# summa-dev/halo2-experiments

Measured on AMD Instinct MI355X. Metric: BN256 G1 MSM throughput, higher is better.
Workload: dtype u32; 1 GPU; standalone BN256 G1 MSM, 2^24 points per GPU (global 2^24 x 1; BASELINE configs[4] microbench, north-star headline size); points_per_gpu=16777216, global_points=16777216, base_set=fixed-base table (registration default from 2^17 points), window_bits=22, windows=12, parallelism=index-range shards x1, all-gather of 96 B partials (RCCL) + host fold, base_set_bytes=12901679104

## Files before the change

halo2-experiments_amd/csrc/ff29.h:

```cpp
#pragma once
#include <stdint.h>

#if defined(__HIPCC__)
#define HM_HD __host__ __device__ __forceinline__
#else
#define HM_HD inline
#endif

#ifdef HM_BOUNDS
#include <cassert>
#include <cmath>
#include <cstdio>
#include <cstdlib>
#define HM_CHECK(cond, what)                                                        \
  do {                                                                              \
    if (!(cond)) {                                                                  \
      std::fprintf(stderr, "HM_BOUNDS violation: %s (%s:%d)\n", what, __FILE__, __LINE__); \
      std::abort();                                                                 \
    }                                                                               \
  } while (0)
#endif

namespace hm {

#include "bn256_constants.inc"

constexpr uint32_t MASK29 = (1u << 29) - 1u;

struct Arr9 {
  uint32_t v[9];
};

template <class F, int K, int BITS>
constexpr Arr9 make_sub_const() {
  Arr9 out{};
  uint64_t carry = 0;
  uint32_t c[9] = {};
  for (int i = 0; i < 9; ++i) {
    uint64_t t = (uint64_t)F::MOD[i] * (uint64_t)K + carry;
    if (i < 8) {
      c[i] = (uint32_t)(t & MASK29);
      carry = t >> 29;
    } else {
      c[i] = (uint32_t)t;
    }
  }
  const uint32_t b = 1u << (BITS - 29);
  out.v[0] = c[0] + (1u << BITS);
  for (int i = 1; i < 8; ++i) out.v[i] = c[i] + (1u << BITS) - b;
  out.v[8] = c[8] - b;
  return out;
}
template <class F, int K, int BITS>
struct SubConst {
  static constexpr Arr9 value = make_sub_const<F, K, BITS>();
};

template <class F>
struct Fe {
  uint32_t l[9];
#ifdef HM_BOUNDS
  double vb = 0;
  uint64_t lb = 0;
  uint64_t tb = 0;
#endif
};

#ifdef HM_BOUNDS
template <class F>
inline double mod_as_double() {
  double m = 0;
  for (int i = 8; i >= 0; --i) m = m * 536870912.0 + (double)F::MOD[i];
  return m;
}
template <class F>
inline uint64_t top_bound_from_value(double vb) {
  return (uint64_t)std::floor(vb * mod_as_double<F>() / std::ldexp(1.0, 232)) + 1;
}
template <class F>
inline void set_bounds(Fe<F>& a, double vb, uint64_t lb, uint64_t tb) {
  a.vb = vb; a.lb = lb; a.tb = tb;
  HM_CHECK(lb < (1ull << 32) && tb < (1ull << 32), "limb bound exceeds 32 bits");
  HM_CHECK(vb * mod_as_double<F>() < std::ldexp(1.0, 261), "value bound exceeds 2^261");
}
// ... 84 lines not shown
  }
#endif
  uint64_t t[10];
#pragma unroll
  for (int j = 0; j < 10; ++j) t[j] = 0;
#pragma unroll
  for (int i = 0; i < 9; ++i) {
#pragma unroll
    for (int j = 0; j < 9; ++j) t[j] += (uint64_t)a.l[j] * b.l[i];
#pragma unroll
    for (int j = 0; j < 9; ++j) t[j] += (uint64_t)c.l[j] * d.l[i];
    const uint32_t m = ((uint32_t)t[0] * F::INV29) & MASK29;
#pragma unroll
    for (int j = 0; j < 9; ++j) t[j] += (uint64_t)m * F::MOD[j];
    t[1] += t[0] >> 29;
#pragma unroll
    for (int j = 0; j < 9; ++j) t[j] = t[j + 1];
    t[9] = 0;
  }
  Fe<F> r;
#pragma unroll
  for (int j = 0; j < 8; ++j) {
    r.l[j] = (uint32_t)t[j] & MASK29;
    t[j + 1] += t[j] >> 29;
  }
  r.l[8] = (uint32_t)t[8];
#ifdef HM_BOUNDS
  {
    double vb = (a.vb * b.vb + c.vb * d.vb) * mod_as_double<F>() / std::ldexp(1.0, 261) + 1.0;
    set_bounds(r, vb, MASK29, top_bound_from_value<F>(vb));
    HM_CHECK(r.l[8] <= r.tb, "fe_mul2 result exceeds its bound");
  }
#endif
  return r;
}

template <class F>
HM_HD Fe<F> fe_sqr(const Fe<F>& a) {
#ifdef HM_BOUNDS
  {
    long double A = (long double)(a.lb > a.tb ? a.lb : a.tb);
    HM_CHECK(2.0L * A < 4294967296.0L, "fe_sqr doubled limb overflows");
    HM_CHECK(9.0L * A * A + 9.0L * 288230376151711744.0L + 1099511627776.0L < 18446744073709551616.0L,
             "fe_sqr column sum may overflow 64 bits");
  }
#endif
  uint32_t d[9];
#pragma unroll
  for (int j = 0; j < 9; ++j) d[j] = a.l[j] << 1;
  uint64_t t[10];
#pragma unroll
  for (int j = 0; j < 10; ++j) t[j] = 0;
#pragma unroll
  for (int i = 0; i < 9; ++i) {
    if (2 * i - i <= 8) t[i] += (uint64_t)a.l[i] * a.l[i];
#pragma unroll
    for (int j = i + 1; j < 9; ++j)
      if (j <= 8) t[j] += (uint64_t)a.l[i] * d[j];
    const uint32_t m = ((uint32_t)t[0] * F::INV29) & MASK29;
#pragma unroll
    for (int j = 0; j < 9; ++j) t[j] += (uint64_t)m * F::MOD[j];
    t[1] += t[0] >> 29;
#pragma unroll
    for (int j = 0; j < 9; ++j) t[j] = t[j + 1];
    t[9] = 0;
  }
  Fe<F> r;
#pragma unroll
  for (int j = 0; j < 8; ++j) {
    r.l[j] = (uint32_t)t[j] & MASK29;
    t[j + 1] += t[j] >> 29;
  }
  r.l[8] = (uint32_t)t[8];
#ifdef HM_BOUNDS
  {
    double vb = a.vb * a.vb * mod_as_double<F>() / std::ldexp(1.0, 261) + 1.0;
    set_bounds(r, vb, MASK29, top_bound_from_value<F>(vb));
    HM_CHECK(r.l[8] <= r.tb, "fe_sqr result exceeds its bound");
  }
#endif
  return r;
}

template <class F>
HM_HD Fe<F> fe_add(const Fe<F>& a, const Fe<F>& b) {
  Fe<F> r;
#pragma unroll
  for (int i = 0; i < 9; ++i) r.l[i] = a.l[i] + b.l[i];
#ifdef HM_BOUNDS
  set_bounds(r, a.vb + b.vb, a.lb + b.lb, a.tb + b.tb);
#endif
  return r;
}

template <class F>
HM_HD Fe<F> fe_dbl(const Fe<F>& a) { return fe_add(a, a); }

template <class F>
HM_HD Fe<F> fe_mul4(const Fe<F>& a) {
  Fe<F> r;
#pragma unroll
  for (int i = 0; i < 9; ++i) r.l[i] = a.l[i] << 2;
#ifdef HM_BOUNDS
  set_bounds(r, 4 * a.vb, 4 * a.lb, 4 * a.tb);
#endif
  return r;
}

template <int K, int BITS, class F>
HM_HD Fe<F> fe_sub(const Fe<F>& a, const Fe<F>& b) {
  constexpr Arr9 S = SubConst<F, K, BITS>::value;
#ifdef HM_BOUNDS
  HM_CHECK(b.lb <= (1ull << BITS) - (1ull << (BITS - 29)), "fe_sub: subtrahend limb bound too large for BITS");
  HM_CHECK(b.tb <= S.v[8], "fe_sub: subtrahend top limb may exceed the constant's");
#endif
  Fe<F> r;
#pragma unroll
  for (int i = 0; i < 9; ++i) r.l[i] = a.l[i] + S.v[i] - b.l[i];
#ifdef HM_BOUNDS
  uint64_t smax = 0;
  for (int i = 0; i < 8; ++i) smax = S.v[i] > smax ? S.v[i] : smax;
  set_bounds(r, a.vb + K, a.lb + smax, a.tb + S.v[8]);
#endif
  return r;
}

template <class F>
HM_HD Fe<F> fe_norm(const Fe<F>& a) {
#ifdef HM_BOUNDS
  HM_CHECK(a.lb + 16 < (1ull << 32) && a.tb + 16 < (1ull << 32), "fe_norm: carry add may overflow");
#endif
  Fe<F> r;
  uint32_t c = 0;
#pragma unroll
  for (int i = 0; i < 8; ++i) {
    const uint32_t t = a.l[i] + c;
    r.l[i] = t & MASK29;
    c = t >> 29;
  }
  r.l[8] = a.l[8] + c;
#ifdef HM_BOUNDS
  set_bounds(r, a.vb, MASK29, top_bound_from_value<F>(a.vb));
  HM_CHECK(r.l[8] <= r.tb, "fe_norm result exceeds its bound");
#endif
  return r;
}

template <class F>
HM_HD bool fe_is_zero_mod(const Fe<F>& a) {
#ifdef HM_BOUNDS
  HM_CHECK(a.lb <= MASK29 && a.vb <= 3.0, "fe_is_zero_mod needs a normalised value < 3*MOD");
#endif
  uint32_t z0 = 0, z1 = 0, z2 = 0;
  uint32_t two[9];
  {
    uint32_t carry = 0;
#pragma unroll
    for (int i = 0; i < 8; ++i) {
      const uint32_t t = 2u * F::MOD[i] + carry;
      two[i] = t & MASK29;
      carry = t >> 29;
    }
    two[8] = 2u * F::MOD[8] + carry;
  }
  if ((a.l[0] != 0u) & (a.l[0] != F::MOD[0]) & (a.l[0] != two[0])) return false;
#pragma unroll
// ... 104 lines not shown
```

halo2-experiments_amd/csrc/g1.h:

```cpp
#pragma once
#include "ff29.h"

namespace hm {

using Fq = Fe<FqParams>;
using Fr = Fe<FrParams>;

struct G1Aff {
  Fq x, y;
};
struct G1Jac {
  Fq x, y, z;
  bool inf;
};

#define HM_G1_XB 12.0
#define HM_G1_YB 5.0
#define HM_G1_ZB 2.0

#ifdef HM_BOUNDS
inline void g1_check_class(const G1Jac& p, const char* what) {
  HM_CHECK(p.x.lb <= MASK29 && p.y.lb <= MASK29 && p.z.lb <= MASK29, what);
  HM_CHECK(p.x.vb <= HM_G1_XB && p.y.vb <= HM_G1_YB && p.z.vb <= HM_G1_ZB, what);
}
// ... 113 lines not shown
    if (fe_is_zero_mod(rr0)) return g1_double_nz(p);
    return g1_identity();
  }
  const Fq i4 = fe_mul4(hh);
  const Fq j = fe_mul(h, i4);
  const Fq r0 = fe_norm(fe_sub<3, 29>(s2, s1));
  const Fq r = fe_dbl(r0);
  const Fq v = fe_mul(u1, i4);
  const Fq rr = fe_sqr(r);
  const Fq t2 = fe_add(j, fe_dbl(v));
  G1Jac o;
  o.x = fe_norm(fe_sub<4, 31>(rr, t2));
  const Fq vx = fe_norm(fe_sub<7, 29>(v, o.x));
  const Fq ns1 = fe_dbl(fe_sub<3, 29>(fe_zero<FqParams>(), s1));
  o.y = fe_mul2(r, vx, ns1, j);
  o.z = fe_mul(fe_mul(p.z, q.z), fe_dbl(h));
  o.inf = false;
  return o;
}

HM_HD G1Jac g1_add(const G1Jac& p, const G1Jac& q) {
  if (p.inf) return q;
  if (q.inf) return p;
  return g1_add_nz(p, q);
}

struct G1Xyzz {
  Fq x, y, zz, zzz;
  bool inf;
};
#define HM_XYZZ_XB 8.0
#define HM_XYZZ_YB 3.0

#ifdef HM_BOUNDS
inline void g1_check_class(const G1Xyzz& p, const char* what) {
  HM_CHECK(p.x.lb <= MASK29 && p.y.lb <= MASK29 && p.zz.lb <= MASK29 && p.zzz.lb <= MASK29, what);
  HM_CHECK(p.x.vb <= HM_XYZZ_XB && p.y.vb <= HM_XYZZ_YB && p.zz.vb <= 2.0 && p.zzz.vb <= 2.0, what);
}
#endif

HM_HD G1Xyzz g1x_identity() {
  G1Xyzz r;
  r.x = fe_zero<FqParams>();
  r.y = fe_zero<FqParams>();
  r.zz = fe_zero<FqParams>();
  r.zzz = fe_zero<FqParams>();
  r.inf = true;
  return r;
}

HM_HD G1Xyzz g1x_from_affine(const G1Aff& p) {
  G1Xyzz r;
  r.x = p.x;
  r.y = p.y;
  r.zz = fe_one<FqParams>();
  r.zzz = fe_one<FqParams>();
  r.inf = false;
  return r;
}

HM_HD G1Jac g1x_to_jac(const G1Xyzz& p) {
  G1Jac r;
  if (p.inf) return g1_identity();
  HM_G1_CHECK(p, "g1x_to_jac input outside class");
  r.x = fe_mul(p.x, fe_sqr(p.zz));
  r.y = fe_mul(p.y, fe_sqr(p.zzz));
  r.z = p.zzz;
  r.inf = false;
  return r;
}

HM_HD G1Xyzz g1x_from_jac(const G1Jac& p) {
  G1Xyzz r;
  if (p.inf) return g1x_identity();
  HM_G1_CHECK(p, "g1x_from_jac input outside class");
  r.zz = fe_sqr(p.z);
  r.zzz = fe_mul(p.z, r.zz);
  r.x = fe_mul(p.x, fe_one<FqParams>());
  r.y = fe_mul(p.y, fe_one<FqParams>());
  r.inf = false;
  return r;
}

HM_HD bool g1x_madd_fast(G1Xyzz& acc, const G1Aff& q, bool neg) {
  HM_G1_CHECK(acc, "g1x_madd_fast input outside class");
  const Fq u2 = fe_mul(q.x, acc.zz);
  const Fq pp0 = fe_norm(fe_sub<9, 29>(u2, acc.x));
  const Fq pp = fe_sqr(pp0);
  if (fe_is_zero_mod(pp)) return false;
  const Fq s2p = fe_mul(q.y, acc.zzz);
  Fq s2;
  {
    const Fq s2n = fe_sub<3, 29>(fe_zero<FqParams>(), s2p);
#pragma unroll
    for (int i = 0; i < 9; ++i) s2.l[i] = neg ? s2n.l[i] : s2p.l[i];
#ifdef HM_BOUNDS
    s2.vb = s2n.vb; s2.lb = s2n.lb; s2.tb = s2n.tb;
#endif
  }
  const Fq r = fe_norm(fe_sub<4, 29>(s2, acc.y));
  const Fq ppp = fe_mul(pp0, pp);
  const Fq qq = fe_mul(acc.x, pp);
  const Fq rr = fe_sqr(r);
  const Fq t2 = fe_add(ppp, fe_dbl(qq));
  const Fq x3 = fe_norm(fe_sub<6, 31>(rr, t2));
  const Fq vx = fe_sub<9, 29>(qq, x3);
  const Fq ny = fe_sub<4, 29>(fe_zero<FqParams>(), acc.y);
  acc.y = fe_mul2(r, vx, ny, ppp);
  acc.x = x3;
  acc.zz = fe_mul(acc.zz, pp);
  acc.zzz = fe_mul(acc.zzz, ppp);
  return true;
}

HM_HD G1Xyzz g1x_madd(const G1Xyzz& p, const G1Aff& q, bool neg = false) {
  if (p.inf) return g1x_from_affine(neg ? g1_neg_affine(q) : q);
  G1Xyzz r = p;
  if (g1x_madd_fast(r, q, neg)) return r;
  return g1x_from_jac(g1_madd_nz(g1x_to_jac(p), q, neg));
}

}
```

halo2-experiments_amd/csrc/host_check.cpp:

```cpp
#include <algorithm>
#include <cstring>
#include <utility>
#include <vector>

#include "g1.h"
#include "graph_lower.h"
#include "host_fr.h"
#include "mock_check.h"

namespace hm {
#include "g1_codec.inc"
#include "poseidon.inc"
#include "keygen.inc"
#include "shplonk.inc"
}

using namespace hm;

namespace {

template <class F>
Fe<F> load_ext(const uint64_t* p) {
  uint32_t w[8];
  std::memcpy(w, p, 32);
// ... 68 lines not shown
GFr gr_reduce(const GFr& lazy) { return fe_reduce_small(fe_norm(lazy)); }
GFr gr_from_ext(const uint32_t* p) {
  uint32_t w[8];
  std::memcpy(w, p, 32);
  return fe_mul(fe_unpack<FrParams>(w), fe_const<FrParams>(FrParams::EXT2INT));
}
GFr gr_from_internal(const uint32_t* p) {
  uint32_t w[8];
  std::memcpy(w, p, 32);
  GFr r = fe_unpack<FrParams>(w);
  HM_DECLARE(r, GE_COLUMN_BOUND);
  return r;
}
const char* g_graph_error = "";

}

extern "C" {

void hc_field_op(int field, int op, const uint64_t* a, const uint64_t* b, uint64_t* o, size_t n) {
  if (field == 0) field_op<FqParams>(op, a, b, o, n);
  else field_op<FrParams>(op, a, b, o, n);
}

void hc_fr_reduce_raw(const uint64_t* a, uint64_t* o, size_t n) {
  for (size_t i = 0; i < n; ++i) {
    uint32_t w[8];
    std::memcpy(w, a + 4 * i, 32);
    Fe<FrParams> x = fe_unpack<FrParams>(w);
    Fe<FrParams> y = fe_canonical(fe_mul(x, fe_const<FrParams>(FrParams::ONE)));
    fe_pack(w, y);
    std::memcpy(o + 4 * i, w, 32);
  }
}

void hc_g1_madd(const uint64_t* pj, int pinf, const uint64_t* q_aff, int neg, uint64_t* out, int* out_inf) {
  G1Jac p = load_jac(pj, pinf);
  G1Aff q;
  q.x = load_ext<FqParams>(q_aff);
  q.y = load_ext<FqParams>(q_aff + 4);
  store_jac(out, out_inf, g1_madd(p, q, neg != 0));
}
void hc_g1_add(const uint64_t* pj, int pinf, const uint64_t* qj, int qinf, uint64_t* out, int* out_inf) {
  store_jac(out, out_inf, g1_add(load_jac(pj, pinf), load_jac(qj, qinf)));
}
void hc_g1_double(const uint64_t* pj, int pinf, uint64_t* out, int* out_inf) {
  store_jac(out, out_inf, g1_double(load_jac(pj, pinf)));
}
void hc_g1_chain(const uint64_t* q_aff, int k, int dbl, uint64_t* out, int* out_inf) {
  G1Aff q;
  q.x = load_ext<FqParams>(q_aff);
  q.y = load_ext<FqParams>(q_aff + 4);
  G1Jac acc = g1_identity();
  for (int i = 0; i < k; ++i) acc = g1_madd(acc, q);
  for (int i = 0; i < dbl; ++i) acc = g1_double(acc);
  store_jac(out, out_inf, acc);
}

void hc_g1x_chain(const uint64_t* q_affs, int k, uint64_t signs, uint64_t* out, int* out_inf) {
  G1Xyzz acc = g1x_identity();
  for (int i = 0; i < k; ++i) {
    G1Aff q;
    q.x = load_ext<FqParams>(q_affs + 8 * i);
    q.y = load_ext<FqParams>(q_affs + 8 * i + 4);
    acc = g1x_madd(acc, q, ((signs >> (i & 63)) & 1) != 0);
  }
  store_jac(out, out_inf, g1x_to_jac(acc));
}

int hc_xyzz_bounds_closure(const uint64_t* pj, const uint64_t* q_aff, double* report) {
  G1Jac pjac = load_jac(pj, 0);
  G1Xyzz p = g1x_from_jac(pjac);
  force_bounds(p.x, HM_XYZZ_XB);
  force_bounds(p.y, HM_XYZZ_YB);
  force_bounds(p.zz, 2.0);
  force_bounds(p.zzz, 2.0);
  G1Aff q;
  q.x = load_ext<FqParams>(q_aff);
  q.y = load_ext<FqParams>(q_aff + 4);
  force_bounds(q.x, 2.0);
  force_bounds(q.y, 2.0);
  G1Xyzz r = p;
  if (!g1x_madd_fast(r, q, true)) return 0;
  const G1Jac j = g1x_to_jac(p);
  report[0] = r.x.vb; report[1] = r.y.vb; report[2] = r.zz.vb; report[3] = r.zzz.vb;
  report[4] = j.x.vb; report[5] = j.y.vb; report[6] = j.z.vb;
  int ok = 1;
  if (r.x.vb > HM_XYZZ_XB || r.y.vb > HM_XYZZ_YB || r.zz.vb > 2.0 || r.zzz.vb > 2.0) ok = 0;
  if (j.x.vb > HM_G1_XB || j.y.vb > HM_G1_YB || j.z.vb > HM_G1_ZB) ok = 0;
  return ok;
}

int hc_bounds_closure(const uint64_t* pj, const uint64_t* qj, const uint64_t* q_aff, double* report) {
  G1Jac p = load_jac(pj, 0), q2 = load_jac(qj, 0);
  at_class_max(p);
  at_class_max(q2);
  G1Aff q;
  q.x = load_ext<FqParams>(q_aff);
  q.y = load_ext<FqParams>(q_aff + 4);
  force_bounds(q.x, 2.0);
  force_bounds(q.y, 2.0);
  G1Jac r[3] = {g1_madd_nz(p, q, true), g1_add_nz(p, q2), g1_double_nz(p)};
  int ok = 1;
  for (int i = 0; i < 3; ++i) {
    report[3 * i + 0] = r[i].x.vb;
    report[3 * i + 1] = r[i].y.vb;
    report[3 * i + 2] = r[i].z.vb;
    if (r[i].x.vb > HM_G1_XB || r[i].y.vb > HM_G1_YB || r[i].z.vb > HM_G1_ZB) ok = 0;
    if (r[i].x.lb > MASK29 || r[i].y.lb > MASK29 || r[i].z.lb > MASK29) ok = 0;
  }
  return ok;
}

int hc_graph_bounds_closure(const uint64_t* a_ext, double* report) {
  typedef Fe<FrParams> F;
  F x = load_ext<FrParams>(a_ext);
  const double CAP = 16.0;
  int ok = 1, r = 0;
  F c16 = x, c16b = x, c3 = x, col = x;
  force_bounds(c16, CAP);
  force_bounds(c16b, CAP);
  force_bounds(c3, 3.0);
  force_bounds(col, 6.0);
  F m = fe_mul(c16, c16b);
  report[r++] = m.vb;
  ok &= m.vb <= 3.0;
  F q = fe_sqr(c16);
  ok &= q.vb <= 3.0;
  ok &= fe_mul(col, c16).vb <= 3.0;
  F h8 = x;
  force_bounds(h8, 8.0);
  F s16 = fe_norm(fe_add(h8, h8));
  report[r++] = s16.vb;
  ok &= s16.vb <= CAP;
  F red = fe_reduce_small(fe_norm(fe_add(c16, c16b)));
  ok &= red.vb <= 3.0;
  F dbl = fe_reduce_small(fe_norm(fe_dbl(c16)));
  ok &= dbl.vb <= 3.0;
  F d12 = x;
  force_bounds(d12, 12.0);
  F sub_lazy = fe_norm(fe_sub<4, 29>(d12, c3));
  report[r++] = sub_lazy.vb;
  ok &= sub_lazy.vb <= CAP;
  ok &= fe_reduce_small(fe_norm(fe_sub<4, 29>(c16, c3))).vb <= 3.0;
  F sub_wide = fe_reduce_small(fe_norm(fe_sub<20, 29>(c16, c16b)));
  report[r++] = sub_wide.vb;
  ok &= sub_wide.vb <= 3.0;
  ok &= fe_reduce_small(fe_norm(fe_sub<20, 29>(fe_zero<FrParams>(), c16))).vb <= 3.0;
  ok &= fe_norm(fe_sub<4, 29>(fe_zero<FrParams>(), c3)).vb <= CAP;
  F d13 = x;
  force_bounds(d13, 13.0);
  F ma = fe_norm(fe_add(fe_mul(c16, c16b), d13));
  report[r++] = ma.vb;
  ok &= ma.vb <= CAP;
  ok &= fe_reduce_small(fe_norm(fe_add(fe_mul(c16, c16b), c16))).vb <= 3.0;
  (void)fe_canonical(fe_mul(fe_reduce_small(fe_norm(c16)), fe_const<FrParams>(FrParams::INT2EXT)));
  return ok;
}

int hc_graph_replay(const uint32_t* calcs5, size_t n_calc, const uint64_t* constants_ext, size_t n_const_static, const uint64_t* dyn_ext,
                    size_t n_dynamic, const int32_t* rotations, size_t n_rot, const uint32_t* const* columns, const uint64_t* column_rows,
                    size_t n_columns, uint32_t n_intermediates, uint32_t log_segment, uint32_t segments, uint32_t flags, uint32_t* values,
                    uint32_t* lowered5, double* static_bound, double* tracked_bound, uint32_t* info) {
  g_graph_error = "";
  if (const char* why = graph_validate(calcs5, n_calc, n_const_static, n_dynamic, n_rot, n_columns, n_intermediates)) {
    g_graph_error = why;
// ... 374 lines not shown
```

halo2-experiments_amd/csrc/msm.hip:

```cpp
#include <hip/hip_runtime.h>

#include <algorithm>
#include <chrono>
#include <cmath>
#include <cstdlib>

#include "hm_internal.h"
#include "host_fq.h"
#include "host_fr.h"
#include "msm_dev.h"

namespace hm {


__global__ void msm_init_counters_kernel(uint32_t* __restrict__ bcnt, size_t nbt, uint32_t* __restrict__ br_count,
                                         uint32_t* __restrict__ khist, uint32_t nkeys, uint32_t* __restrict__ big_count) {
  const size_t i0 = (size_t)blockIdx.x * blockDim.x + threadIdx.x, stride = (size_t)gridDim.x * blockDim.x;
  for (size_t i = i0; i < nbt; i += stride) bcnt[i] = 0;
  if (i0 < nkeys) khist[i0] = 0;
  if (i0 < 4) {
    if (br_count) br_count[i0] = 0;
    big_count[i0] = 0;
  }
}
// ... 1003 lines not shown
}

__global__ __launch_bounds__(ORDER_THREADS) void msm_task_keyscan_kernel(const uint32_t* __restrict__ khist,
                                                                         uint32_t* __restrict__ kcursor) {
  __shared__ uint32_t s[TASK_KEYS];
  const uint32_t tid = threadIdx.x, v = khist[tid];
  s[tid] = v;
  __syncthreads();
  for (uint32_t off = 1; off < TASK_KEYS; off <<= 1) {
    const uint32_t a = tid >= off ? s[tid - off] : 0u;
    __syncthreads();
    s[tid] += a;
    __syncthreads();
  }
  kcursor[tid] = s[tid] - v;
}

__global__ __launch_bounds__(ORDER_THREADS) void msm_task_order_kernel(const uint32_t* __restrict__ bcnt,
                                                                       const uint32_t* __restrict__ toff, uint32_t NBT,
                                                                       const uint32_t* __restrict__ pairs, uint32_t L_host,
                                                                       uint32_t* __restrict__ kcursor,
                                                                       uint32_t* __restrict__ task_bucket,
                                                                       uint32_t* __restrict__ task_order,
                                                                       const uint32_t* __restrict__ totals) {
  __shared__ uint32_t h[TASK_KEYS], base[TASK_KEYS];
  if (totals[2]) return;
  const uint32_t L = effective_task_len(pairs, L_host);
  h[threadIdx.x] = 0;
  __syncthreads();
  uint32_t cnt[ORDER_ITEMS];
#pragma unroll
  for (int k = 0; k < ORDER_ITEMS; ++k) {
    const uint32_t b = (blockIdx.x * ORDER_ITEMS + k) * ORDER_THREADS + threadIdx.x;
    cnt[k] = b < NBT ? bcnt[b] : 0u;
    const uint32_t full = cnt[k] / L, rem = cnt[k] - full * L;
    if (full) atomicAdd(&h[task_key(L, L)], full);
    if (rem) atomicAdd(&h[task_key(rem, L)], 1u);
  }
  __syncthreads();
  {
    const uint32_t mine = h[threadIdx.x];
    base[threadIdx.x] = mine ? atomicAdd(&kcursor[threadIdx.x], mine) : 0u;
    h[threadIdx.x] = 0;
  }
  __syncthreads();
  __shared__ uint32_t hot_n, hot[ORDER_HOT][4];
  if (threadIdx.x == 0) hot_n = 0;
  __syncthreads();
#pragma unroll
  for (int k = 0; k < ORDER_ITEMS; ++k) {
    const uint32_t b = (blockIdx.x * ORDER_ITEMS + k) * ORDER_THREADS + threadIdx.x;
    if (cnt[k] == 0) continue;
    const uint32_t full = cnt[k] / L, rem = cnt[k] - full * L;
    const uint32_t t0 = toff[b];
    if (full) {
      const uint32_t key = task_key(L, L), at = base[key] + atomicAdd(&h[key], full);
      const uint32_t slot = full > 64 ? atomicAdd(&hot_n, 1u) : ORDER_HOT;
      if (slot < ORDER_HOT) {
        hot[slot][0] = b; hot[slot][1] = t0; hot[slot][2] = full; hot[slot][3] = at;
      } else {
        for (uint32_t i = 0; i < full; ++i) {
          task_bucket[t0 + i] = b;
          task_order[at + i] = t0 + i;
        }
      }
    }
    if (rem) {
      const uint32_t key = task_key(rem, L);
      task_bucket[t0 + full] = b;
      task_order[base[key] + atomicAdd(&h[key], 1u)] = t0 + full;
    }
  }
  __syncthreads();
  const uint32_t nh = hot_n < ORDER_HOT ? hot_n : ORDER_HOT;
  for (uint32_t e = 0; e < nh; ++e) {
    const uint32_t b = hot[e][0], t0 = hot[e][1], full = hot[e][2], at = hot[e][3];
    for (uint32_t i = threadIdx.x; i < full; i += ORDER_THREADS) {
      task_bucket[t0 + i] = b;
      task_order[at + i] = t0 + i;
    }
  }
}

#ifdef HM_K3_WAVES
#define HM_K3_OCC __attribute__((amdgpu_waves_per_eu(HM_K3_WAVES, HM_K3_WAVES)))
#else
#define HM_K3_OCC
#endif
__global__ __launch_bounds__(ACC_THREADS) HM_K3_OCC void msm_accumulate_kernel(const uint32_t* __restrict__ sorted,
                                                                     const uint32_t* __restrict__ task_bucket,
                                                                     const uint32_t* __restrict__ task_order,
                                                                     const uint32_t* __restrict__ boff,
                                                                     const uint32_t* __restrict__ bcnt,
                                                                     const uint32_t* __restrict__ toff,
                                                                     const uint32_t* __restrict__ xy,
                                                                     uint32_t* __restrict__ partial,
                                                                     const uint32_t* __restrict__ totals,
                                                                     const uint32_t* __restrict__ pairs, uint32_t L_host) {
  __shared__ uint4 stage[4][ACC_THREADS];
  const uint32_t L = effective_task_len(pairs, L_host);
  const uint32_t lane = threadIdx.x;
  const uint32_t slot = blockIdx.x * ACC_THREADS + lane;
  const uint32_t T = totals[1];
  uint32_t start = 0, end = 0, t = 0;
  if (slot < T) {
    t = task_order[slot];
    const uint32_t b = task_bucket[t];
    const uint32_t k = t - toff[b];
    start = boff[b] + k * L;
    const uint32_t bucket_end = boff[b] + bcnt[b];
    end = start + L < bucket_end ? start + L : bucket_end;
  }
  if (start >= end) return;
  const G1Jac res = accumulate_chain(sorted, xy, start, end, stage, lane);
  store_jac(partial + (size_t)t * PT_WORDS, res);
}


constexpr uint32_t FINALIZE_SERIAL = 8;
constexpr uint32_t FINALIZE_SLICE = 2048;
__global__ __launch_bounds__(ACC_THREADS) void msm_bucket_finalize_kernel(const uint32_t* __restrict__ partial,
                                                                          const uint32_t* __restrict__ toff,
                                                                          uint32_t* __restrict__ bucket, uint32_t NBT,
                                                                          uint32_t* __restrict__ big_count,
                                                                          uint32_t* __restrict__ big_list,
                                                                          uint2* __restrict__ slice_list,
                                                                          const uint32_t* __restrict__ totals) {
  const uint32_t b = blockIdx.x * ACC_THREADS + threadIdx.x;
  if (b >= NBT) return;
  if (totals[2]) {
    store_jac(bucket + (size_t)b * PT_WORDS, g1_identity());
    return;
  }
  const uint32_t lo = toff[b], hi = toff[b + 1];
  if (hi - lo > FINALIZE_SERIAL) {
    big_list[atomicAdd(big_count, 1u)] = b;
    if (hi - lo > FINALIZE_SLICE) {
      const uint32_t nsl = (hi - lo + FINALIZE_SLICE - 1) / FINALIZE_SLICE;
      const uint32_t at = atomicAdd(big_count + 1, nsl);
      for (uint32_t k = 0; k < nsl; ++k) slice_list[at + k] = make_uint2(b, k);
    }
    return;
  }
  G1Jac acc = g1_identity();
  for (uint32_t t = lo; t < hi; ++t) acc = g1_add(acc, load_jac(partial + (size_t)t * PT_WORDS));
  store_jac(bucket + (size_t)b * PT_WORDS, acc);
}

__global__ __launch_bounds__(WIN_THREADS) void msm_bucket_finalize_slices_kernel(uint32_t* __restrict__ partial,
                                                                                 const uint32_t* __restrict__ toff,
                                                                                 const uint32_t* __restrict__ big_count,
                                                                                 const uint2* __restrict__ slice_list) {
  __shared__ uint32_t tree[WIN_THREADS * PT_WORDS];
  const uint32_t count = big_count[1];
  for (uint32_t item = blockIdx.x; item < count; item += gridDim.x) {
    const uint2 e = slice_list[item];
    const uint32_t lo = toff[e.x] + e.y * FINALIZE_SLICE;
    const uint32_t end = toff[e.x + 1], hi = lo + FINALIZE_SLICE < end ? lo + FINALIZE_SLICE : end;
    G1Jac acc = g1_identity();
    for (uint32_t t = lo + threadIdx.x; t < hi; t += WIN_THREADS) acc = g1_add(acc, load_jac(partial + (size_t)t * PT_WORDS));
    const G1Jac r = block_sum_points(tree, acc);
    if (threadIdx.x == 0) store_jac(partial + (size_t)lo * PT_WORDS, r);
    __syncthreads();
  }
}

__global__ __launch_bounds__(WIN_THREADS) void msm_bucket_finalize_big_kernel(const uint32_t* __restrict__ partial,
                                                                              const uint32_t* __restrict__ toff,
                                                                              uint32_t* __restrict__ bucket,
                                                                              const uint32_t* __restrict__ big_count,
                                                                              const uint32_t* __restrict__ big_list) {
  __shared__ uint32_t tree[WIN_THREADS * PT_WORDS];
  const uint32_t count = *big_count;
  for (uint32_t item = blockIdx.x; item < count; item += gridDim.x) {
    const uint32_t b = big_list[item];
    const uint32_t lo = toff[b], hi = toff[b + 1];
    const uint32_t step = hi - lo > FINALIZE_SLICE ? FINALIZE_SLICE : 1u;
    G1Jac acc = g1_identity();
    for (uint32_t t = lo + threadIdx.x * step; t < hi; t += WIN_THREADS * step)
      acc = g1_add(acc, load_jac(partial + (size_t)t * PT_WORDS));
    const G1Jac r = block_sum_points(tree, acc);
    if (threadIdx.x == 0) store_jac(bucket + (size_t)b * PT_WORDS, r);
    __syncthreads();
  }
}

__global__ __launch_bounds__(ACC_THREADS) void msm_reduce_segments_kernel(const uint32_t* __restrict__ bucket,
                                                                          uint32_t* __restrict__ segres, uint32_t W,
                                                                          uint32_t NB, uint32_t NBP, uint32_t SEG,
                                                                          uint32_t nseg) {
  const uint32_t idx = blockIdx.x * ACC_THREADS + threadIdx.x;
  if (idx >= W * nseg) return;
  const uint32_t w = idx / nseg, sgi = idx - w * nseg;
  const uint32_t lo = sgi * SEG + 1;
  const uint32_t hi = lo + SEG - 1 < NB ? lo + SEG - 1 : NB;
  const uint32_t* bw = bucket + (size_t)w * NBP * PT_WORDS;
  G1Jac run = g1_identity(), acc = g1_identity();
// ... 1060 lines not shown
```

halo2-experiments_amd/csrc/msm_dev.h:

```cpp
#pragma once
#include <hip/hip_runtime.h>

#include "g1.h"

namespace hm {

constexpr int PT_WORDS = 28;

__device__ __forceinline__ G1Jac load_jac(const uint32_t* p) {
  const uint4* q = reinterpret_cast<const uint4*>(p);
  uint32_t w[PT_WORDS];
#pragma unroll
  for (int i = 0; i < 7; ++i) {
    const uint4 v = q[i];
    w[4 * i] = v.x; w[4 * i + 1] = v.y; w[4 * i + 2] = v.z; w[4 * i + 3] = v.w;
  }
  G1Jac r;
#pragma unroll
  for (int i = 0; i < 9; ++i) {
    r.x.l[i] = w[i];
    r.y.l[i] = w[9 + i];
    r.z.l[i] = w[18 + i];
  }
  r.inf = w[27] != 0;
  return r;
}
__device__ __forceinline__ void store_jac(uint32_t* p, const G1Jac& a) {
  uint32_t w[PT_WORDS];
#pragma unroll
  for (int i = 0; i < 9; ++i) {
    w[i] = a.x.l[i];
    w[9 + i] = a.y.l[i];
    w[18 + i] = a.z.l[i];
  }
  w[27] = a.inf ? 1u : 0u;
  uint4* q = reinterpret_cast<uint4*>(p);
#pragma unroll
  for (int i = 0; i < 7; ++i) q[i] = make_uint4(w[4 * i], w[4 * i + 1], w[4 * i + 2], w[4 * i + 3]);
}

__device__ __forceinline__ G1Aff load_base(const uint32_t* xy, uint32_t idx) {
  const uint4* q = reinterpret_cast<const uint4*>(xy + (size_t)idx * 16);
  const uint4 a = q[0], b = q[1], c = q[2], d = q[3];
  const uint32_t wx[8] = {a.x, a.y, a.z, a.w, b.x, b.y, b.z, b.w};
  const uint32_t wy[8] = {c.x, c.y, c.z, c.w, d.x, d.y, d.z, d.w};
  G1Aff r;
  r.x = fe_unpack<FqParams>(wx);
  r.y = fe_unpack<FqParams>(wy);
  return r;
}

constexpr int ACC_THREADS = 64;

typedef __attribute__((address_space(3))) void hm_lds_void;
typedef __attribute__((address_space(1))) const void hm_gbl_void;

__device__ __forceinline__ void stage_base_async(const uint32_t* xy, uint32_t idx, uint4 (*stage)[ACC_THREADS]) {
  const uint4* src = reinterpret_cast<const uint4*>(xy + (size_t)idx * 16);
#pragma unroll
  for (int k = 0; k < 4; ++k)
    __builtin_amdgcn_global_load_lds((hm_gbl_void*)(src + k), (hm_lds_void*)&stage[k][0], 16, 0, 0);
}

__device__ __forceinline__ G1Jac accumulate_chain(const uint32_t* __restrict__ sorted, const uint32_t* __restrict__ xy,
                                                  uint32_t start, uint32_t end, uint4 (*stage)[ACC_THREADS], uint32_t lane) {
  uint32_t v_cur = sorted[start];
  G1Xyzz acc;
  {
    const G1Aff q0 = load_base(xy, v_cur & 0x7fffffffu);
    acc = g1x_from_affine((v_cur >> 31) ? g1_neg_affine(q0) : q0);
  }
  uint32_t p = start + 1, v_next = 0;
  if (p < end) {
    v_cur = sorted[p];
    stage_base_async(xy, v_cur & 0x7fffffffu, stage);
    if (p + 1 < end) v_next = sorted[p + 1];
  }
  bool general = false;
  for (; p < end; ++p) {
    asm volatile("s_waitcnt vmcnt(0)" ::: "memory");
    const uint4 a = stage[0][lane], b4 = stage[1][lane], c4 = stage[2][lane], d4 = stage[3][lane];
    asm volatile("s_waitcnt lgkmcnt(0)" ::: "memory");
    const bool neg = (v_cur >> 31) != 0;
    if (p + 1 < end) {
      v_cur = v_next;
      stage_base_async(xy, v_cur & 0x7fffffffu, stage);
      if (p + 2 < end) v_next = sorted[p + 2];
    }
    const uint32_t wx[8] = {a.x, a.y, a.z, a.w, b4.x, b4.y, b4.z, b4.w};
    const uint32_t wy[8] = {c4.x, c4.y, c4.z, c4.w, d4.x, d4.y, d4.z, d4.w};
    G1Aff q;
    q.x = fe_unpack<FqParams>(wx);
    q.y = fe_unpack<FqParams>(wy);
    if (!g1x_madd_fast(acc, q, neg)) {
      general = true;
      break;
    }
  }
  asm volatile("s_waitcnt vmcnt(0)" ::: "memory");
  G1Jac res = g1x_to_jac(acc);
  if (general) {
    for (; p < end; ++p) {
      const uint32_t v = sorted[p];
      res = g1_madd(res, load_base(xy, v & 0x7fffffffu), (v >> 31) != 0);
    }
  }
  return res;
}

constexpr int WIN_THREADS = 256;
__device__ __forceinline__ G1Jac block_sum_points(uint32_t* tree, G1Jac acc) {
  const uint32_t t = threadIdx.x;
  store_jac(tree + t * PT_WORDS, acc);
  __syncthreads();
  for (uint32_t off = WIN_THREADS / 2; off > 0; off >>= 1) {
    if (t < off) {
      const G1Jac a = load_jac(tree + t * PT_WORDS), b = load_jac(tree + (t + off) * PT_WORDS);
      store_jac(tree + t * PT_WORDS, g1_add(a, b));
    }
    __syncthreads();
  }
  return load_jac(tree);
}


__device__ __forceinline__ uint32_t lds_inc(uint32_t* cnt, uint32_t bin) {
#ifndef HM_NO_AGG
  const uint32_t v = (uint32_t)__builtin_amdgcn_readfirstlane((int)bin);
  const uint64_t active = __ballot(1);
  if (__ballot(bin == v) == active) {
    const uint32_t lane = __builtin_amdgcn_mbcnt_hi(~0u, __builtin_amdgcn_mbcnt_lo(~0u, 0u));
    const uint32_t before = (uint32_t)__popcll(active & ((1ull << lane) - 1ull));
    uint32_t base = 0;
    if (before == 0) base = atomicAdd(&cnt[v], (uint32_t)__popcll(active));
    base = (uint32_t)__builtin_amdgcn_readfirstlane((int)base);
    return base + before;
  }
#endif
  return atomicAdd(&cnt[bin], 1u);
}

__device__ __forceinline__ G1Jac block_sum_points_upto(uint32_t* tree, G1Jac acc, uint32_t count) {
  const uint32_t t = threadIdx.x;
  uint32_t top = 1;
  while (top < count) top <<= 1;
  if (t < top) store_jac(tree + t * PT_WORDS, acc);
  __syncthreads();
  for (uint32_t off = top / 2; off > 0; off >>= 1) {
    if (t < off) {
      const G1Jac a = load_jac(tree + t * PT_WORDS), b = load_jac(tree + (t + off) * PT_WORDS);
      store_jac(tree + t * PT_WORDS, g1_add(a, b));
    }
    __syncthreads();
  }
  return load_jac(tree);
}

__device__ __forceinline__ void store_window_ext(uint32_t* o, const G1Jac& r) {
  uint32_t wx[8], wy[8], wz[8];
  if (r.inf) {
#pragma unroll
    for (int k = 0; k < 8; ++k) wx[k] = wy[k] = wz[k] = 0;
  } else {
    fe_to_ext(wx, r.x);
    fe_to_ext(wy, r.y);
    fe_to_ext(wz, r.z);
  }
#pragma unroll
  for (int k = 0; k < 8; ++k) {
    o[k] = wx[k];
    o[8 + k] = wy[k];
    o[16 + k] = wz[k];
  }
  o[24] = r.inf ? 1u : 0u;
}

}
// ... 1 lines not shown
```

Baseline: 930.7 million points/s.

## Interleave independent Montgomery products in lockstep within XYZZ mixed addition

Adds lockstep Montgomery multiply and square helpers that run two or three independent field products column by column with interleaved accumulators. The XYZZ mixed-add used by the bucket accumulate kernel is reordered to group independent multiplications, aiming to expose instruction-level parallelism and hide multiply latency. The accumulate kernel is also pinned to a fixed waves-per-EU occupancy of 4 by default. This raises register pressure and moves the zero check after the squarings, so degenerate cases do some extra work before bailing out.

```diff
diff --git a/halo2-experiments_amd/csrc/ff29.h b/halo2-experiments_amd/csrc/ff29.h
--- a/halo2-experiments_amd/csrc/ff29.h
+++ b/halo2-experiments_amd/csrc/ff29.h
@@ -1,5 +1,7 @@
 #pragma once
 #include <stdint.h>
+
+#include <utility>
 
 #if defined(__HIPCC__)
 #define HM_HD __host__ __device__ __forceinline__
@@ -250,6 +252,183 @@
   return r;
 }
 
+#if defined(__HIP_DEVICE_COMPILE__) && !defined(HM_BOUNDS)
+#define HM_PIN(x) asm("" : "+v"(x))
+#else
+#define HM_PIN(x) ((void)0)
+#endif
+
+template <class F>
+struct MontMul {
+  const Fe<F>&a, &b;
+  HM_HD static constexpr int terms(int k) { return (k < 8 ? k : 8) - (k > 8 ? k - 8 : 0) + 1; }
+  HM_HD uint64_t term(int k, int s) const {
+    const int i = (k > 8 ? k - 8 : 0) + s;
+    return (uint64_t)a.l[i] * b.l[k - i];
+  }
+};
+template <class F>
+struct MontMul2 {
+  const Fe<F>&a, &b, &c, &d;
+  HM_HD static constexpr int terms(int k) { return 2 * MontMul<F>::terms(k); }
+  HM_HD uint64_t term(int k, int s) const {
+    const int n = MontMul<F>::terms(k), i = (k > 8 ? k - 8 : 0) + (s < n ? s : s - n);
+    return s < n ? (uint64_t)a.l[i] * b.l[k - i] : (uint64_t)c.l[i] * d.l[k - i];
+  }
+};
+template <class F>
+struct MontSqr {
+  const Fe<F>& a;
+  const uint32_t (&d)[9];
+  HM_HD static constexpr int pairs(int k) { return (k + 1) / 2 - (k > 8 ? k - 8 : 0); }
+  HM_HD static constexpr int terms(int k) { return pairs(k) + (k % 2 == 0 ? 1 : 0); }
+  HM_HD uint64_t term(int k, int s) const {
+    const int i = (k > 8 ? k - 8 : 0) + s;
+    return s < pairs(k) ? (uint64_t)a.l[i] * d[k - i] : (uint64_t)a.l[k / 2] * a.l[k / 2];
+  }
+};
+
+template <class F, class P>
+struct MontLane {
+  P p;
+  uint64_t acc;
+  uint32_t m[9];
+  Fe<F> r;
+};
+template <class F, class P>
+HM_HD void mont_step_ab(MontLane<F, P>& L, int k, int s) {
+  if (s < P::terms(k)) {
+    L.acc += L.p.term(k, s);
+    HM_PIN(L.acc);
+  }
+}
+template <class F, class P>
+HM_HD void mont_step_mp(MontLane<F, P>& L, int k, int i) {
+  L.acc += (uint64_t)L.m[i] * F::MOD[k - i];
+  HM_PIN(L.acc);
+}
+template <class F, class P>
+HM_HD void mont_step_end(MontLane<F, P>& L, int k) {
+  if (k < 9) {
+    L.m[k] = ((uint32_t)L.acc * F::INV29) & MASK29;
+    L.acc += (uint64_t)L.m[k] * F::MOD[0];
+    HM_PIN(L.acc);
+  } else {
+    L.r.l[k - 9] = (uint32_t)L.acc & MASK29;
+  }
+  L.acc >>= 29;
+  HM_PIN(L.acc);
+}
+template <int K, class F, class... P>
+HM_HD void mont_column(MontLane<F, P>&... L) {
+#pragma unroll
+  for (int s = 0; s < 18; ++s) (mont_step_ab(L, K, s), ...);
+#pragma unroll
+  for (int i = (K > 8 ? K - 8 : 0); i <= (K < 8 ? K - 1 : 8); ++i) (mont_step_mp(L, K, i), ...);
+  (mont_step_end(L, K), ...);
+}
+template <class F, int... Ks, class... P>
+HM_HD void mont_columns(std::integer_sequence<int, Ks...>, MontLane<F, P>&... L) {
+  (mont_column<Ks, F>(L...), ...);
+}
+template <class F, class... P>
+HM_HD void mont_run(MontLane<F, P>&... L) {
+  ((L.acc = 0), ...);
+  mont_columns<F>(std::make_integer_sequence<int, 17>{}, L...);
+  ((L.r.l[8] = (uint32_t)L.acc), ...);
+}
+
+#ifdef HM_BOUNDS
+template <class F>
+inline long double fe_limb_max(const Fe<F>& a) { return (long double)(a.lb > a.tb ? a.lb : a.tb); }
+inline void mont_check_column(long double sum_ab, const char* what) {
+  HM_CHECK(9.0L * sum_ab + 9.0L * 288230376151711744.0L + 1099511627776.0L < 18446744073709551616.0L, what);
+}
+template <class F>
+inline void mont_set_result(Fe<F>& r, double vb_products, const char* what) {
+  const double vb = vb_products * mod_as_double<F>() / std::ldexp(1.0, 261) + 1.0;
+  set_bounds(r, vb, MASK29, top_bound_from_value<F>(vb));
+  HM_CHECK(r.l[8] <= r.tb, what);
+}
+#define HM_MUL_PRE(a, b) mont_check_column(fe_limb_max(a) * fe_limb_max(b), "fe_mul column sum may overflow 64 bits")
+#define HM_MUL_POST(r, a, b) mont_set_result(r, (a).vb * (b).vb, "fe_mul result exceeds its bound")
+#define HM_MUL2_PRE(a, b, c, d) \
+  mont_check_column(fe_limb_max(a) * fe_limb_max(b) + fe_limb_max(c) * fe_limb_max(d), "fe_mul2 column sum may overflow 64 bits")
+#define HM_MUL2_POST(r, a, b, c, d) mont_set_result(r, (a).vb * (b).vb + (c).vb * (d).vb, "fe_mul2 result exceeds its bound")
+#define HM_SQR_PRE(a)                                                                   \
+  do {                                                                                  \
+    HM_CHECK(2.0L * fe_limb_max(a) < 4294967296.0L, "fe_sqr doubled limb overflows");   \
+    mont_check_column(fe_limb_max(a) * fe_limb_max(a), "fe_sqr column sum may overflow 64 bits"); \
+  } while (0)
+#define HM_SQR_POST(r, a) mont_set_result(r, (a).vb * (a).vb, "fe_sqr result exceeds its bound")
+#else
+#define HM_MUL_PRE(a, b) ((void)0)
+#define HM_MUL_POST(r, a, b) ((void)0)
+#define HM_MUL2_PRE(a, b, c, d) ((void)0)
+#define HM_MUL2_POST(r, a, b, c, d) ((void)0)
+#define HM_SQR_PRE(a) ((void)0)
+#define HM_SQR_POST(r, a) ((void)0)
+#endif
+
+template <class F>
+HM_HD void fe_doubled_limbs(uint32_t (&d)[9], const Fe<F>& a) {
+#pragma unroll
+  for (int j = 0; j < 9; ++j) d[j] = a.l[j] << 1;
+}
+template <class F>
+HM_HD void fe_mul_x2(Fe<F>& r0, Fe<F>& r1, const Fe<F>& a0, const Fe<F>& b0, const Fe<F>& a1, const Fe<F>& b1) {
+  HM_MUL_PRE(a0, b0);
+  HM_MUL_PRE(a1, b1);
+  MontLane<F, MontMul<F>> L0{{a0, b0}}, L1{{a1, b1}};
+  mont_run<F>(L0, L1);
+  HM_MUL_POST(L0.r, a0, b0);
+  HM_MUL_POST(L1.r, a1, b1);
+  r0 = L0.r;
+  r1 = L1.r;
+}
+template <class F>
+HM_HD void fe_mul_x3(Fe<F>& r0, Fe<F>& r1, Fe<F>& r2, const Fe<F>& a0, const Fe<F>& b0, const Fe<F>& a1, const Fe<F>& b1,
+                     const Fe<F>& a2, const Fe<F>& b2) {
+  HM_MUL_PRE(a0, b0);
+  HM_MUL_PRE(a1, b1);
+  HM_MUL_PRE(a2, b2);
+  MontLane<F, MontMul<F>> L0{{a0, b0}}, L1{{a1, b1}}, L2{{a2, b2}};
+  mont_run<F>(L0, L1, L2);
+  HM_MUL_POST(L0.r, a0, b0);
+  HM_MUL_POST(L1.r, a1, b1);
+  HM_MUL_POST(L2.r, a2, b2);
+  r0 = L0.r;
+  r1 = L1.r;
+  r2 = L2.r;
+}
+template <class F>
+HM_HD void fe_sqr_x2(Fe<F>& r0, Fe<F>& r1, const Fe<F>& a0, const Fe<F>& a1) {
+  HM_SQR_PRE(a0);
+  HM_SQR_PRE(a1);
+  uint32_t d0[9], d1[9];
+  fe_doubled_limbs(d0, a0);
+  fe_doubled_limbs(d1, a1);
+  MontLane<F, MontSqr<F>> L0{{a0, d0}}, L1{{a1, d1}};
+  mont_run<F>(L0, L1);
+  HM_SQR_POST(L0.r, a0);
+  HM_SQR_POST(L1.r, a1);
+  r0 = L0.r;
+  r1 = L1.r;
+}
+template <class F>
+HM_HD void fe_mul_mul2(Fe<F>& r0, Fe<F>& r1, const Fe<F>& a0, const Fe<F>& b0, const Fe<F>& a, const Fe<F>& b, const Fe<F>& c,
+                       const Fe<F>& d) {
+  HM_MUL_PRE(a0, b0);
+  HM_MUL2_PRE(a, b, c, d);
+  MontLane<F, MontMul<F>> L0{{a0, b0}};
+  MontLane<F, MontMul2<F>> L1{{a, b, c, d}};
+  mont_run<F>(L0, L1);
+  HM_MUL_POST(L0.r, a0, b0);
+  HM_MUL2_POST(L1.r, a, b, c, d);
+  r0 = L0.r;
+  r1 = L1.r;
+}
+
 template <class F>
 HM_HD Fe<F> fe_add(const Fe<F>& a, const Fe<F>& b) {
   Fe<F> r;
diff --git a/halo2-experiments_amd/csrc/g1.h b/halo2-experiments_amd/csrc/g1.h
--- a/halo2-experiments_amd/csrc/g1.h
+++ b/halo2-experiments_amd/csrc/g1.h
@@ -219,13 +219,21 @@
   return r;
 }
 
+template <bool LOCKSTEP = false>
 HM_HD bool g1x_madd_fast(G1Xyzz& acc, const G1Aff& q, bool neg) {
   HM_G1_CHECK(acc, "g1x_madd_fast input outside class");
-  const Fq u2 = fe_mul(q.x, acc.zz);
+  Fq u2, s2p, pp, rr, ppp, qq, zz3, zzz3, y3;
+  if constexpr (LOCKSTEP) {
+    fe_mul_x2(u2, s2p, q.x, acc.zz, q.y, acc.zzz);
+  } else {
+    u2 = fe_mul(q.x, acc.zz);
+  }
   const Fq pp0 = fe_norm(fe_sub<9, 29>(u2, acc.x));
-  const Fq pp = fe_sqr(pp0);
-  if (fe_is_zero_mod(pp)) return false;
-  const Fq s2p = fe_mul(q.y, acc.zzz);
+  if constexpr (!LOCKSTEP) {
+    pp = fe_sqr(pp0);
+    if (fe_is_zero_mod(pp)) return false;
+    s2p = fe_mul(q.y, acc.zzz);
+  }
   Fq s2;
   {
     const Fq s2n = fe_sub<3, 29>(fe_zero<FqParams>(), s2p);
@@ -236,17 +244,30 @@
 #endif
   }
   const Fq r = fe_norm(fe_sub<4, 29>(s2, acc.y));
-  const Fq ppp = fe_mul(pp0, pp);
-  const Fq qq = fe_mul(acc.x, pp);
-  const Fq rr = fe_sqr(r);
+  if constexpr (LOCKSTEP) {
+    fe_sqr_x2(pp, rr, pp0, r);
+    if (fe_is_zero_mod(pp)) return false;
+    fe_mul_x3(ppp, qq, zz3, pp0, pp, acc.x, pp, acc.zz, pp);
+  } else {
+    ppp = fe_mul(pp0, pp);
+    qq = fe_mul(acc.x, pp);
+    rr = fe_sqr(r);
+  }
   const Fq t2 = fe_add(ppp, fe_dbl(qq));
   const Fq x3 = fe_norm(fe_sub<6, 31>(rr, t2));
   const Fq vx = fe_sub<9, 29>(qq, x3);
   const Fq ny = fe_sub<4, 29>(fe_zero<FqParams>(), acc.y);
-  acc.y = fe_mul2(r, vx, ny, ppp);
+  if constexpr (LOCKSTEP) {
+    fe_mul_mul2(zzz3, y3, acc.zzz, ppp, r, vx, ny, ppp);
+  } else {
+    y3 = fe_mul2(r, vx, ny, ppp);
+    zz3 = fe_mul(acc.zz, pp);
+    zzz3 = fe_mul(acc.zzz, ppp);
+  }
   acc.x = x3;
-  acc.zz = fe_mul(acc.zz, pp);
-  acc.zzz = fe_mul(acc.zzz, ppp);
+  acc.y = y3;
+  acc.zz = zz3;
+  acc.zzz = zzz3;
   return true;
 }
 
diff --git a/halo2-experiments_amd/csrc/host_check.cpp b/halo2-experiments_amd/csrc/host_check.cpp
--- a/halo2-experiments_amd/csrc/host_check.cpp
+++ b/halo2-experiments_amd/csrc/host_check.cpp
@@ -174,6 +174,13 @@
   force_bounds(q.y, 2.0);
   G1Xyzz r = p;
   if (!g1x_madd_fast(r, q, true)) return 0;
+  {
+    G1Xyzz rl = p;
+    if (!g1x_madd_fast<true>(rl, q, true)) return 0;
+    for (int i = 0; i < 9; ++i)
+      if (rl.x.l[i] != r.x.l[i] || rl.y.l[i] != r.y.l[i] || rl.zz.l[i] != r.zz.l[i] || rl.zzz.l[i] != r.zzz.l[i]) return 0;
+    if (rl.x.vb > HM_XYZZ_XB || rl.y.vb > HM_XYZZ_YB || rl.zz.vb > 2.0 || rl.zzz.vb > 2.0) return 0;
+  }
   const G1Jac j = g1x_to_jac(p);
   report[0] = r.x.vb; report[1] = r.y.vb; report[2] = r.zz.vb; report[3] = r.zzz.vb;
   report[4] = j.x.vb; report[5] = j.y.vb; report[6] = j.z.vb;
diff --git a/halo2-experiments_amd/csrc/msm.hip b/halo2-experiments_amd/csrc/msm.hip
--- a/halo2-experiments_amd/csrc/msm.hip
+++ b/halo2-experiments_amd/csrc/msm.hip
@@ -1109,11 +1109,10 @@
   }
 }
 
-#ifdef HM_K3_WAVES
+#ifndef HM_K3_WAVES
+#define HM_K3_WAVES 4
+#endif
 #define HM_K3_OCC __attribute__((amdgpu_waves_per_eu(HM_K3_WAVES, HM_K3_WAVES)))
-#else
-#define HM_K3_OCC
-#endif
 __global__ __launch_bounds__(ACC_THREADS) HM_K3_OCC void msm_accumulate_kernel(const uint32_t* __restrict__ sorted,
                                                                      const uint32_t* __restrict__ task_bucket,
                                                                      const uint32_t* __restrict__ task_order,
@@ -1139,7 +1138,7 @@
     end = start + L < bucket_end ? start + L : bucket_end;
   }
   if (start >= end) return;
-  const G1Jac res = accumulate_chain(sorted, xy, start, end, stage, lane);
+  const G1Jac res = accumulate_chain<true>(sorted, xy, start, end, stage, lane);
   store_jac(partial + (size_t)t * PT_WORDS, res);
 }
 
diff --git a/halo2-experiments_amd/csrc/msm_dev.h b/halo2-experiments_amd/csrc/msm_dev.h
--- a/halo2-experiments_amd/csrc/msm_dev.h
+++ b/halo2-experiments_amd/csrc/msm_dev.h
@@ -62,6 +62,7 @@
     __builtin_amdgcn_global_load_lds((hm_gbl_void*)(src + k), (hm_lds_void*)&stage[k][0], 16, 0, 0);
 }
 
+template <bool LOCKSTEP = false>
 __device__ __forceinline__ G1Jac accumulate_chain(const uint32_t* __restrict__ sorted, const uint32_t* __restrict__ xy,
                                                   uint32_t start, uint32_t end, uint4 (*stage)[ACC_THREADS], uint32_t lane) {
   uint32_t v_cur = sorted[start];
@@ -92,7 +93,7 @@
     G1Aff q;
     q.x = fe_unpack<FqParams>(wx);
     q.y = fe_unpack<FqParams>(wy);
-    if (!g1x_madd_fast(acc, q, neg)) {
+    if (!g1x_madd_fast<LOCKSTEP>(acc, q, neg)) {
       general = true;
       break;
     }
```

Result: faster. 965.1 million points/s, median of 6 (+3.7%).
